# sevagh/Zen

Hardware: AMD Instinct MI355X
Metric: hops/sec (1024-hop HPR, 44.1 kHz mono) (higher is better)
Workload: dtype f32

## Files before the change

zen_amd/blockrun/blockrun_kernel.hip:

```cpp
#include "../csrc/common.h"
#include "../csrc/fft_dev.h"
#include "../csrc/masks.h"
#include "../csrc/median47_core.h"
#include "../csrc/median_net.h"
#include "blockrun_kernel.h"
#include "blockrun_first_pass.h"
#include "blockrun_edge_count.h"

#pragma clang fp contract(off)

namespace zen_blockrun {
namespace {

using zen_hip_impl::hard_mask_exact;
using PL = zfft::Plan<12>;
constexpr int N = PL::N, TF = PL::TF;
static_assert(N == NFFT && TF == 256 && HOP == 4 * TF, "four samples of a hop per thread");

constexpr int MID = TAPS / 2, MID_AL = 24, IMG_END = 255 * 16 + 64;
__device__ __forceinline__ int img_addr(int g) { return (g >> 4) * zm47::RSTR + (g & 15); }
constexpr int MIR_LO = 56, MIR_HI = 39;
static_assert(N - MIR_LO <= 16 * 254 - 24 && N / 2 + MIR_HI >= 16 * 128 + 39, "blocks 254 / 255 and 126 .. 128 read written columns");
static_assert(EDGE_IMG_COL0 == MID_AL && EDGE_IMG_RSTR == zm47::RSTR && EDGE_OUTPUTS == MID + 1, "blockrun_edge_count.h reads this image");
constexpr int PC_WORD = 5184, PC_TAIL = 2052, EDGE_WORD = PC_WORD + PC_TAIL + 512 + 4;
static_assert((EDGE_WORD + 256) * 4 <= PL::LDS_FLOAT2 * 8, "lean layout must fit in the frame image");
constexpr int KEEP_WORD = PL::LDS_FLOAT2 * 2, CARRY_WORD = KEEP_WORD + HOP, WIN_WORD = CARRY_WORD + HOP;
constexpr size_t LDS_BYTES = (size_t)(WIN_WORD + 2 * HOP) * 4;
static_assert(LDS_BYTES <= LDS_BYTES_MAX, "three workgroups per CU");

__device__ __forceinline__ void lds_barrier()
{
	asm volatile("s_waitcnt lgkmcnt(0)\n\ts_barrier" ::: "memory");
}

struct TwGlobal32 {
	static constexpr bool PLAIN = true;
	static constexpr bool PACKED = true;
	const float2* __restrict__ p;
	__device__ __forceinline__ float2 get(int, int, int, int idx) const
	{
		return *reinterpret_cast<const float2*>(reinterpret_cast<const char*>(p) + (unsigned)(idx << 3));
	}
};

struct Spec {
	float2 S[16];
};

struct FwdInPre {
	float x[8], w[8];
	__device__ __forceinline__ float2 operator()(int, int slot) const { return make_float2(x[slot] * w[slot], 0.0f); }
};

struct FwdOut {
	Spec* r;
	int* img;
	__device__ __forceinline__ void operator()(int idx, float2 X, bool lower, int slot) const
	{
		r->S[slot] = X;
		if (slot == 8) {
			if (__builtin_amdgcn_readfirstlane(idx) < (N >> 1) + 64 && idx == (N >> 1))
				img[img_addr((N >> 1) + MID_AL)] = __float_as_int(zfft::cabs_exact(X.x, X.y));
		}
		else if (lower) {
			const float m = zfft::cabs_exact(X.x, X.y);
			const int key = __float_as_int(m);
			constexpr int CH = (TF / 16) * zm47::RSTR;
			const int tfl = idx - slot * TF;
			img[img_addr(tfl + MID_AL) + slot * CH] = key;
			if (slot == 0 && tfl >= 1 && tfl <= MIR_LO)
				img[img_addr(N - tfl + MID_AL)] = key;
			if (slot == 7 && tfl >= TF - MIR_HI)
				img[img_addr(N - 7 * TF - tfl + MID_AL)] = key;
		}
	}
};

struct InvIn {
	const Spec* r;
	const int* img;
	const float* pc;
	double thr;
	__device__ __forceinline__ float2 operator()(int idx, int slot) const
	{
		const int lo = slot * TF, hi = lo + TF - 1;
		int pi;
		if (hi <= N / 2)
			pi = idx;
		else if (lo > N / 2 && hi < N - MID)
			pi = N - idx;
		else
			pi = (idx > N / 2 && idx < N - MID) ? N - idx : (idx > N / 2 ? idx - (N - 512) + PC_TAIL : idx);
		const int g0 = hi <= N / 2 ? idx + 24 - slot * TF : TF + 24 - (idx - slot * TF);
		const float mag = __int_as_float(img[(g0 >> 4) * 20 + (g0 & 15) + (hi <= N / 2 ? slot : 15 - slot) * (TF / 16) * 20]);
		const float2 z = r->S[slot];
		const float p = pc[pi];
		float m = hard_mask_exact(p, mag + FLT_EPSILON, thr);
		if (hi > N / 2 && !(lo > N / 2 && hi < N - MID))
			m = (idx == N / 2 || idx >= N - MID) ? p : m;
		return make_float2(z.x * m, z.y * m);
	}
};

struct InvOut {
	float* Y;
	float* out;
	float* carry;
	float cola;
	__device__ __forceinline__ void operator()(int idx, float2 x, bool, int slot) const
	{
		const float y = x.x * cola;
		ZH_CHK(Y + idx, 1);
		Y[idx] = y;
		if (slot < 4) {
			ZH_CHK(out + idx, 1);
			out[idx] = carry[(slot & 3) * TF] + y;
		}
		else {
			carry[(slot & 3) * TF] = y;
		}
	}
};

template <bool SYM>
__device__ __forceinline__ void run_body(const RunArgs& a)
{
	extern __shared__ float2 lds[];
	int* img = reinterpret_cast<int*>(lds);
	float* Prow = reinterpret_cast<float*>(img + PC_WORD);
	const int tf = (int)threadIdx.x;
	float* keep = reinterpret_cast<float*>(img + KEEP_WORD) + tf;
	float* carry = reinterpret_cast<float*>(img + CARRY_WORD) + tf;
	float* win = reinterpret_cast<float*>(img + WIN_WORD) + tf;

	int s, f0, len;
	zen_blockrun_run(&a.part, (int)blockIdx.x, &s, &f0, &len);
	if (s >= a.n_streams || f0 + len > a.n_frames)
		return;
	const float* cur = a.in + (long long)s * a.in_stride + (long long)f0 * HOP;
	float* Yrow = a.Y + (long long)s * a.y_stream_stride + (long long)f0 * (2 * HOP);
	float* orow = a.out + (long long)s * a.out_stride + (long long)f0 * HOP;

	if (a.prev_frames > 0) {
		const int fc = a.prev_frames - 1 < a.n_frames - 1 ? a.prev_frames - 1 : a.n_frames - 1;
		if (fc >= f0 && fc < f0 + len) {
			const float* y = a.Y + (long long)s * a.y_stream_stride + (long long)(a.prev_frames - 1) * (2 * HOP) + HOP;
			float v[4];
#pragma unroll
			for (int i = 0; i < 4; ++i) {
				ZH_CHK(y + tf + i * TF, 1);
				v[i] = y[tf + i * TF];
			}
#pragma unroll
			for (int i = 0; i < 4; ++i) {
				ZH_CHK(a.carry + ((long long)s * HOP + tf + i * TF), 1);
				a.carry[(long long)s * HOP + tf + i * TF] = v[i];
			}
		}
	}
	float nx[4];
	{
		const float* pv = f0 > 0 ? cur - HOP : a.tail_prev + (long long)s * HOP;
		float p[4], w[8];
#pragma unroll
		for (int m = 0; m < 4; ++m) {
			ZH_CHK(pv + m * TF + tf, 1);
			ZH_CHK(cur + m * TF + tf, 1);
			p[m] = pv[m * TF + tf];
			nx[m] = cur[m * TF + tf];
		}
#pragma unroll
		for (int m = 0; m < 8; ++m) {
			ZH_CHK(a.window + m * TF + tf, 1);
			w[m] = a.window[m * TF + tf];
		}
#pragma unroll
		for (int m = 0; m < 4; ++m) {
			keep[m * TF] = p[m];
			carry[m * TF] = 0.0f;
		}
#pragma unroll
		for (int m = 0; m < 8; ++m)
			win[m * TF] = w[m];
	}
	if (tf == 0) {
		ZH_CHK(a.need + ((long long)s * a.n_frames + f0), 1);
		a.need[(long long)s * a.n_frames + f0] = 1u;
	}

	const int tf_run = tf;
	for (int k = 0; k < len; ++k) {
		const int f = f0 + k;
		int tf = tf_run, tw_off = 0;
		asm volatile("" : "+v"(tf));
		tf &= TF - 1;
		asm volatile("" : "+s"(tw_off));
		const float2* tw = a.tw + tw_off;
		float* keep = reinterpret_cast<float*>(img + KEEP_WORD) + tf;
		float* carry = reinterpret_cast<float*>(img + CARRY_WORD) + tf;
		float* win = reinterpret_cast<float*>(img + WIN_WORD) + tf;
		Spec r;
		{
			FwdInPre pre;
#pragma unroll
			for (int m = 0; m < 4; ++m) {
				pre.x[m] = keep[m * TF];
				pre.x[4 + m] = nx[m];
			}
#pragma unroll
			for (int m = 0; m < 8; ++m)
				pre.w[m] = win[m * TF];
#pragma unroll
			for (int m = 0; m < 4; ++m)
				keep[m * TF] = nx[m];
			if (f == a.n_frames - 1) {
				float* tail = a.tail_next + (long long)s * HOP;
#pragma unroll
				for (int m = 0; m < 4; ++m) {
					ZH_CHK(tail + m * TF + tf, 1);
					tail[m * TF + tf] = nx[m];
				}
			}
			FwdOut out;
			out.r = &r;
			out.img = img;
			{
				float p[8];
#pragma unroll
				for (int m = 0; m < 8; ++m)
					p[m] = pre.x[m] * pre.w[m];
				float2 Y0[16];
				first_pass16<true, SYM>(p, a.tw16, a.tw8, a.tw3_16, Y0);
#pragma unroll
				for (int c = 0; c < 16; ++c)
					lds[PL::pad_off(tf, c * (N / 16))] = Y0[c];
				zfft::frame_sync<TF>();
			}
			zfft::PassRunner<12, 1, false, true, false, FwdInPre, FwdOut, false, TwGlobal32>::run(tf, lds, TwGlobal32{tw}, pre, out, true);
		}
		lds_barrier();
		if (f >= a.n_frames - a.keep_mag_rows) {
			float* mag = a.mag + (((a.row0 + f) % a.ring_rows) + (long long)s * a.ring_rows) * N;
			for (int g = tf; g < N; g += TF) {
				ZH_CHK(mag + g, 1);
				mag[g] = __int_as_float(img[img_addr((g <= N / 2 ? g : N - g) + MID_AL)]);
			}
		}
		{
			const int v0 = img[img_addr(MID_AL)], v1 = img[img_addr(N - 1 + MID_AL)];
			for (int g = tf; g < MID_AL; g += TF)
				img[img_addr(g)] = v0;
			for (int g = N + MID_AL + tf; g < IMG_END; g += TF)
				img[img_addr(g)] = v1;
		}
		lds_barrier();
		{
			int(*edge)[64] = reinterpret_cast<int(*)[64]>(img + EDGE_WORD);
			const int lane = tf & 63, wave = __builtin_amdgcn_readfirstlane(tf >> 6);
			zm47::Pieces pc;
			if (wave < 3) {
				zm47::m47_sort_and_publish(img, edge, tf, lane, wave, tf == 0, false, pc);
			}
			else {
				const unsigned bits = edge_count_wave(img, lane, a.thr, N / 2);
				if (lane < EDGE_OUTPUTS)
					Prow[lane == 0 ? N / 2 : PC_TAIL + 512 - lane] = (bits >> lane) & 1u ? 1.0f : 0.0f;
			}
			lds_barrier();
			if (wave < 2) {
				int o[16];
				zm47::m47_select(img, edge, tf, wave, pc, o);
#pragma unroll
				for (int v = 0; v < 4; ++v)
					*reinterpret_cast<int4*>(&Prow[tf * 16 + 4 * v]) = make_int4(o[4 * v], o[4 * v + 1], o[4 * v + 2], o[4 * v + 3]);
			}
		}
		lds_barrier();
		cur += HOP;
		if (k + 1 < len) {
#pragma unroll
			for (int m = 0; m < 4; ++m) {
				ZH_CHK(cur + m * TF + tf, 1);
				nx[m] = cur[m * TF + tf];
			}
		}
		{
			asm volatile("" : "+v"(tf));
			asm volatile("" : "+s"(tw_off));
			tf &= TF - 1;
			tw = a.tw + tw_off;
			carry = reinterpret_cast<float*>(img + CARRY_WORD) + tf;
			InvIn in;
			in.r = &r;
			in.img = img;
			in.pc = Prow;
			in.thr = a.thr;
			InvOut out;
			out.Y = Yrow;
			out.out = orow;
			out.carry = carry;
			out.cola = a.cola;
			zfft::PassRunner<12, 0, true, false, true, InvIn, InvOut, true, TwGlobal32>::run(tf, lds, TwGlobal32{tw}, in, out, true);
		}
		Yrow += 2 * HOP;
		orow += HOP;
	}
}

__global__ __launch_bounds__(256, 3) void blockrun_kernel(RunArgs a) { run_body<true>(a); }
__global__ __launch_bounds__(256, 3) void blockrun_kernel_plain_table(RunArgs a) { run_body<false>(a); }

__global__ __launch_bounds__(256) void blockrun_fixup_kernel(RunArgs a)
{
	const long long total = (long long)a.n_streams * a.n_frames;
	const long long item = (long long)blockIdx.x * 4 + (threadIdx.x >> 6);
	const int lane = threadIdx.x & 63;
	if (item >= total)
		return;
	ZH_CHK(a.need + item, 1);
	if (!a.need[item])
		return;
	const int s = (int)(item / a.n_frames), f = (int)(item - (long long)s * a.n_frames);
	const float* Y = a.Y + (long long)s * a.y_stream_stride + (long long)f * (2 * HOP);
	const float* prev = f == 0 ? a.carry + (long long)s * HOP : Y - HOP;
	float* o = a.out + (long long)s * a.out_stride + (long long)f * HOP;
	if (((reinterpret_cast<uintptr_t>(o) | reinterpret_cast<uintptr_t>(prev) | reinterpret_cast<uintptr_t>(Y)) & 15) == 0) {
		float4 p[HOP / 256], y[HOP / 256];
#pragma unroll
		for (int i = 0; i < HOP / 256; ++i) {
			const int k = i * 256 + lane * 4;
			ZH_CHK(prev + k, 4);
			ZH_CHK(Y + k, 4);
			p[i] = *reinterpret_cast<const float4*>(prev + k);
			y[i] = *reinterpret_cast<const float4*>(Y + k);
		}
#pragma unroll
		for (int i = 0; i < HOP / 256; ++i) {
			const int k = i * 256 + lane * 4;
			ZH_CHK(o + k, 4);
			*reinterpret_cast<float4*>(o + k) = make_float4(p[i].x + y[i].x, p[i].y + y[i].y, p[i].z + y[i].z, p[i].w + y[i].w);
		}
	}
	else {
		for (int k = lane; k < HOP; k += 64) {
			ZH_CHK(o + k, 1);
			ZH_CHK(prev + k, 1);
			ZH_CHK(Y + k, 1);
			o[k] = prev[k] + Y[k];
		}
	}
	if (lane == 0)
		a.need[item] = 0u;
}

}

size_t run_kernel_lds_bytes() { return LDS_BYTES; }

int launch_run(const RunArgs& a, hipStream_t stream)
{
	const long long runs = (long long)a.n_streams * a.part.runs_per_stream;
	if (a.tw_symmetric)
		hipLaunchKernelGGL(blockrun_kernel, dim3((unsigned)runs), dim3(TF), LDS_BYTES, stream, a);
	else
		hipLaunchKernelGGL(blockrun_kernel_plain_table, dim3((unsigned)runs), dim3(TF), LDS_BYTES, stream, a);
	ZH_HIP(hipGetLastError());
	return ZEN_HIP_OK;
}

int launch_fixup(const RunArgs& a, hipStream_t stream)
{
	const long long total = (long long)a.n_streams * a.n_frames;
	hipLaunchKernelGGL(blockrun_fixup_kernel, dim3((unsigned)((total + 3) / 4)), dim3(256), 0, stream, a);
	ZH_HIP(hipGetLastError());
	return ZEN_HIP_OK;
}

}
```

Before: 62.44 million.

## Precompute hard mask row in LDS and use real-output inverse FFT last pass

Moves the hard-mask evaluation out of the inverse FFT input functor into a separate vectorized pass over the mask row, so the inverse FFT reads a single precomputed mask value per bin. The image border fill is now done by one lane during the forward output, which removes a separate fill loop and one barrier. The generic inverse FFT runner is replaced by a specialized routine whose last pass computes only the eight real outputs that are needed, using split even/odd radix-8 butterflies. In exchange it adds a new barrier after mask computation and carries the risk of subtle indexing errors in the custom last pass.

```diff
diff --git a/zen_amd/blockrun/blockrun_image.h b/zen_amd/blockrun/blockrun_image.h
--- /dev/null
+++ b/zen_amd/blockrun/blockrun_image.h
@@ -0,0 +1,23 @@
+#pragma once
+#include <hip/hip_runtime.h>
+
+namespace zen_blockrun {
+
+constexpr int IMG_N = 4096, IMG_TF = 256;
+constexpr int IMG_COL0 = 24, IMG_RSTR = 20;
+constexpr int IMG_MIR_HI = 39;
+constexpr int IMG_BORDER_STORES = 6;
+constexpr int IMG_WORDS = ((IMG_N + 2 * IMG_COL0) / 16) * IMG_RSTR;
+
+#define ZBR_IMG_FN __device__ __forceinline__
+
+ZBR_IMG_FN int img_addr(int g) { return (g >> 4) * IMG_RSTR + (g & 15); }
+ZBR_IMG_FN int img_col(int col) { return img_addr(col + IMG_COL0); }
+ZBR_IMG_FN int img_own(int tfl, int slot) { return img_col(tfl) + slot * (IMG_TF / 16) * IMG_RSTR; }
+ZBR_IMG_FN bool img_mirrored(int tfl, int slot) { return slot == 7 && tfl >= IMG_TF - IMG_MIR_HI; }
+ZBR_IMG_FN int img_mirror(int tfl) { return img_col(IMG_N - 7 * IMG_TF - tfl); }
+ZBR_IMG_FN int img_border(int i) { return i < 4 ? 4 * i : IMG_RSTR + 4 * (i - 4); }
+
+static_assert(IMG_N / 2 + IMG_MIR_HI >= 16 * 128 + 39, "blocks 126 .. 129 read written columns");
+
+}
diff --git a/zen_amd/blockrun/blockrun_kernel.hip b/zen_amd/blockrun/blockrun_kernel.hip
--- a/zen_amd/blockrun/blockrun_kernel.hip
+++ b/zen_amd/blockrun/blockrun_kernel.hip
@@ -5,7 +5,9 @@
 #include "../csrc/median_net.h"
 #include "blockrun_kernel.h"
 #include "blockrun_first_pass.h"
+#include "blockrun_last_pass.h"
 #include "blockrun_edge_count.h"
+#include "blockrun_image.h"
 
 #pragma clang fp contract(off)
 
@@ -17,12 +19,11 @@
 constexpr int N = PL::N, TF = PL::TF;
 static_assert(N == NFFT && TF == 256 && HOP == 4 * TF, "four samples of a hop per thread");
 
-constexpr int MID = TAPS / 2, MID_AL = 24, IMG_END = 255 * 16 + 64;
-__device__ __forceinline__ int img_addr(int g) { return (g >> 4) * zm47::RSTR + (g & 15); }
-constexpr int MIR_LO = 56, MIR_HI = 39;
-static_assert(N - MIR_LO <= 16 * 254 - 24 && N / 2 + MIR_HI >= 16 * 128 + 39, "blocks 254 / 255 and 126 .. 128 read written columns");
-static_assert(EDGE_IMG_COL0 == MID_AL && EDGE_IMG_RSTR == zm47::RSTR && EDGE_OUTPUTS == MID + 1, "blockrun_edge_count.h reads this image");
+constexpr int MID = TAPS / 2;
+static_assert(IMG_N == N && IMG_TF == TF && IMG_COL0 == 24 && IMG_RSTR == zm47::RSTR, "blockrun_image.h describes this image");
+static_assert(EDGE_IMG_COL0 == IMG_COL0 && EDGE_IMG_RSTR == zm47::RSTR && EDGE_OUTPUTS == MID + 1, "blockrun_edge_count.h reads this image");
 constexpr int PC_WORD = 5184, PC_TAIL = 2052, EDGE_WORD = PC_WORD + PC_TAIL + 512 + 4;
+static_assert(PC_WORD >= IMG_WORDS, "the mask row lies behind the image");
 static_assert((EDGE_WORD + 256) * 4 <= PL::LDS_FLOAT2 * 8, "lean layout must fit in the frame image");
 constexpr int KEEP_WORD = PL::LDS_FLOAT2 * 2, CARRY_WORD = KEEP_WORD + HOP, WIN_WORD = CARRY_WORD + HOP;
 constexpr size_t LDS_BYTES = (size_t)(WIN_WORD + 2 * HOP) * 4;
@@ -60,27 +61,30 @@
 		r->S[slot] = X;
 		if (slot == 8) {
 			if (__builtin_amdgcn_readfirstlane(idx) < (N >> 1) + 64 && idx == (N >> 1))
-				img[img_addr((N >> 1) + MID_AL)] = __float_as_int(zfft::cabs_exact(X.x, X.y));
+				img[img_col(N >> 1)] = __float_as_int(zfft::cabs_exact(X.x, X.y));
 		}
 		else if (lower) {
 			const float m = zfft::cabs_exact(X.x, X.y);
 			const int key = __float_as_int(m);
-			constexpr int CH = (TF / 16) * zm47::RSTR;
 			const int tfl = idx - slot * TF;
-			img[img_addr(tfl + MID_AL) + slot * CH] = key;
-			if (slot == 0 && tfl >= 1 && tfl <= MIR_LO)
-				img[img_addr(N - tfl + MID_AL)] = key;
-			if (slot == 7 && tfl >= TF - MIR_HI)
-				img[img_addr(N - 7 * TF - tfl + MID_AL)] = key;
+			img[img_own(tfl, slot)] = key;
+			if (slot == 0) {
+				if (__builtin_amdgcn_readfirstlane(idx) < 64 && idx == 0) {
+					const int4 q = make_int4(key, key, key, key);
+#pragma unroll
+					for (int i = 0; i < IMG_BORDER_STORES; ++i)
+						*reinterpret_cast<int4*>(&img[img_border(i)]) = q;
+				}
+			}
+			if (img_mirrored(tfl, slot))
+				img[img_mirror(tfl)] = key;
 		}
 	}
 };
 
 struct InvIn {
 	const Spec* r;
-	const int* img;
 	const float* pc;
-	double thr;
 	__device__ __forceinline__ float2 operator()(int idx, int slot) const
 	{
 		const int lo = slot * TF, hi = lo + TF - 1;
@@ -91,13 +95,8 @@
 			pi = N - idx;
 		else
 			pi = (idx > N / 2 && idx < N - MID) ? N - idx : (idx > N / 2 ? idx - (N - 512) + PC_TAIL : idx);
-		const int g0 = hi <= N / 2 ? idx + 24 - slot * TF : TF + 24 - (idx - slot * TF);
-		const float mag = __int_as_float(img[(g0 >> 4) * 20 + (g0 & 15) + (hi <= N / 2 ? slot : 15 - slot) * (TF / 16) * 20]);
 		const float2 z = r->S[slot];
-		const float p = pc[pi];
-		float m = hard_mask_exact(p, mag + FLT_EPSILON, thr);
-		if (hi > N / 2 && !(lo > N / 2 && hi < N - MID))
-			m = (idx == N / 2 || idx >= N - MID) ? p : m;
+		const float m = pc[pi];
 		return make_float2(z.x * m, z.y * m);
 	}
 };
@@ -127,7 +126,7 @@
 {
 	extern __shared__ float2 lds[];
 	int* img = reinterpret_cast<int*>(lds);
-	float* Prow = reinterpret_cast<float*>(img + PC_WORD);
+	float* Mrow = reinterpret_cast<float*>(img + PC_WORD);
 	const int tf = (int)threadIdx.x;
 	float* keep = reinterpret_cast<float*>(img + KEEP_WORD) + tf;
 	float* carry = reinterpret_cast<float*>(img + CARRY_WORD) + tf;
@@ -243,17 +242,9 @@
 			float* mag = a.mag + (((a.row0 + f) % a.ring_rows) + (long long)s * a.ring_rows) * N;
 			for (int g = tf; g < N; g += TF) {
 				ZH_CHK(mag + g, 1);
-				mag[g] = __int_as_float(img[img_addr((g <= N / 2 ? g : N - g) + MID_AL)]);
-			}
-		}
-		{
-			const int v0 = img[img_addr(MID_AL)], v1 = img[img_addr(N - 1 + MID_AL)];
-			for (int g = tf; g < MID_AL; g += TF)
-				img[img_addr(g)] = v0;
-			for (int g = N + MID_AL + tf; g < IMG_END; g += TF)
-				img[img_addr(g)] = v1;
-		}
-		lds_barrier();
+				mag[g] = __int_as_float(img[img_col(g <= N / 2 ? g : N - g)]);
+			}
+		}
 		{
 			int(*edge)[64] = reinterpret_cast<int(*)[64]>(img + EDGE_WORD);
 			const int lane = tf & 63, wave = __builtin_amdgcn_readfirstlane(tf >> 6);
@@ -264,7 +255,7 @@
 			else {
 				const unsigned bits = edge_count_wave(img, lane, a.thr, N / 2);
 				if (lane < EDGE_OUTPUTS)
-					Prow[lane == 0 ? N / 2 : PC_TAIL + 512 - lane] = (bits >> lane) & 1u ? 1.0f : 0.0f;
+					Mrow[lane == 0 ? N / 2 : PC_TAIL + 512 - lane] = (bits >> lane) & 1u ? 1.0f : 0.0f;
 			}
 			lds_barrier();
 			if (wave < 2) {
@@ -272,7 +263,7 @@
 				zm47::m47_select(img, edge, tf, wave, pc, o);
 #pragma unroll
 				for (int v = 0; v < 4; ++v)
-					*reinterpret_cast<int4*>(&Prow[tf * 16 + 4 * v]) = make_int4(o[4 * v], o[4 * v + 1], o[4 * v + 2], o[4 * v + 3]);
+					*reinterpret_cast<int4*>(&Mrow[tf * 16 + 4 * v]) = make_int4(o[4 * v], o[4 * v + 1], o[4 * v + 2], o[4 * v + 3]);
 			}
 		}
 		lds_barrier();
@@ -284,6 +275,22 @@
 				nx[m] = cur[m * TF + tf];
 			}
 		}
+		{
+			float* pm = Mrow + tf * 8;
+			const int* hm = img + img_col(tf * 8);
+#pragma unroll
+			for (int v = 0; v < 2; ++v) {
+				const float4 p = *reinterpret_cast<const float4*>(pm + 4 * v);
+				const int4 h = *reinterpret_cast<const int4*>(hm + 4 * v);
+				float4 q;
+				q.x = hard_mask_exact(p.x, __int_as_float(h.x) + FLT_EPSILON, a.thr);
+				q.y = hard_mask_exact(p.y, __int_as_float(h.y) + FLT_EPSILON, a.thr);
+				q.z = hard_mask_exact(p.z, __int_as_float(h.z) + FLT_EPSILON, a.thr);
+				q.w = hard_mask_exact(p.w, __int_as_float(h.w) + FLT_EPSILON, a.thr);
+				*reinterpret_cast<float4*>(pm + 4 * v) = q;
+			}
+		}
+		lds_barrier();
 		{
 			asm volatile("" : "+v"(tf));
 			asm volatile("" : "+s"(tw_off));
@@ -292,15 +299,17 @@
 			carry = reinterpret_cast<float*>(img + CARRY_WORD) + tf;
 			InvIn in;
 			in.r = &r;
-			in.img = img;
-			in.pc = Prow;
-			in.thr = a.thr;
+			in.pc = Mrow;
 			InvOut out;
 			out.Y = Yrow;
 			out.out = orow;
 			out.carry = carry;
 			out.cola = a.cola;
+#ifdef ZBR_GENERIC_LAST_PASS
 			zfft::PassRunner<12, 0, true, false, true, InvIn, InvOut, true, TwGlobal32>::run(tf, lds, TwGlobal32{tw}, in, out, true);
+#else
+			inverse_real_half(tf, lds, TwGlobal32{tw}, in, out);
+#endif
 		}
 		Yrow += 2 * HOP;
 		orow += HOP;
diff --git a/zen_amd/blockrun/blockrun_last_pass.h b/zen_amd/blockrun/blockrun_last_pass.h
--- /dev/null
+++ b/zen_amd/blockrun/blockrun_last_pass.h
@@ -0,0 +1,78 @@
+#pragma once
+#include "../csrc/fft_dev.h"
+
+#pragma clang fp contract(off)
+
+namespace zen_blockrun {
+
+template <class TW>
+__device__ __forceinline__ void last_pass_real8(const float2 (&a)[16], int k, int log2L, int log2N, const TW& tw, int pass, float (&y)[8])
+{
+	float2 ev[8], od[8];
+#pragma unroll
+	for (int i = 0; i < 8; ++i) {
+		ev[i] = a[2 * i];
+		od[i] = a[2 * i + 1];
+	}
+	zfft::butterfly<8, true, false, false, TW>(ev, k, log2L, log2N, tw, pass, 0);
+	zfft::butterfly<8, true, false, false, TW>(od, k, log2L, log2N, tw, pass, 0);
+	float2 w[8];
+#pragma unroll
+	for (int c = 0; c < 8; ++c) {
+		if (c >= 4) {
+			w[c] = make_float2(-w[c - 4].y, w[c - 4].x);
+		}
+		else {
+			const float2 t = tw.get(pass, 0, 4 + c, (k << (log2N - log2L - 4)) + (c << (log2N - 4)));
+			w[c] = make_float2(t.x, -t.y);
+		}
+	}
+#pragma unroll
+	for (int c = 0; c < 8; ++c) {
+		const float t = w[c].x * od[c].x - w[c].y * od[c].y;
+		y[c] = ev[c].x + t;
+	}
+}
+
+template <class In, class Out, class TW>
+__device__ __forceinline__ void inverse_real_half(int tf, float2* __restrict__ lds, const TW& tw, In& in, Out& out)
+{
+	using PL = zfft::Plan<12>;
+	constexpr int N = PL::N, TF = PL::TF;
+	static_assert(PL::P == 3 && PL::r(0) == 4 && PL::r(1) == 4 && PL::r(2) == 4 && PL::V == 16 && !PL::INPLACE, "three passes of 16 values");
+	float2 v[16];
+#pragma unroll
+	for (int m = 0; m < 16; ++m)
+		v[m] = in(m * TF + tf, m);
+	zfft::frame_sync<TF>();
+	zfft::butterfly<16, true, false, TW::PLAIN, TW>(v, 0, 0, 12, tw, 0, 0);
+#pragma unroll
+	for (int c = 0; c < 16; ++c)
+		lds[PL::pad_off(tf, c * (N / 16))] = v[c];
+	zfft::frame_sync<TF>();
+	{
+		const int k = tf >> 4, j = tf & 15;
+#pragma unroll
+		for (int m = 0; m < 16; ++m)
+			v[m] = lds[PL::pad_off(k * 256 + j, m * 16)];
+		zfft::frame_sync<TF>();
+		zfft::butterfly<16, true, false, false, TW>(v, k, 4, 12, tw, 1, 0);
+#pragma unroll
+		for (int c = 0; c < 16; ++c)
+			lds[PL::pad_off(tf, c * (N / 16))] = v[c];
+		zfft::frame_sync<TF>();
+	}
+	{
+#pragma unroll
+		for (int m = 0; m < 16; ++m)
+			v[m] = lds[PL::pad_off(tf * 16, m)];
+		zfft::frame_sync<TF>();
+		float y[8];
+		last_pass_real8(v, tf, 8, 12, tw, 2, y);
+#pragma unroll
+		for (int c = 0; c < 8; ++c)
+			out(tf + c * (N / 16), make_float2(y[c], 0.0f), true, c);
+	}
+}
+
+}
```

Result: no change. 63.04 million (median of 6 runs) (+1.0%).
